# SiyuanHuang95/SUG

Measured on AMD Instinct MI355X. Metric: point-clouds/sec (train step, N=1024), higher is better.
Workload: dtype f32

## Files before the change

include/sug_amd.h:

```cpp
#ifndef SUG_AMD_H
#define SUG_AMD_H

#include <stdint.h>

#ifdef __cplusplus
extern "C" {
#endif

#define SUG_OK 0
#define SUG_ERR_ARG (-1)
#define SUG_ERR_LAUNCH (-2)
#define SUG_STATS_BLOCKS 1024

const char* sug_last_error(void);
#define SUG_ABI_VERSION 7
int sug_abi_version(void);

int sug_knn(const float* x, int64_t ldx, int B, int N, int C, int k,
            int32_t* idx, void* stream);

int sug_knn_reverse(const int32_t* idx, int B, int N, int k,
                    int32_t* rev_off, int32_t* rev_ent, void* stream);

int sug_fps(const float* xyz, const int32_t* start, int B, int N, int npoint,
            int32_t* out, void* stream);

int sug_ball_query(const float* xyz, const float* query, int B, int N, int S,
                   float r2, int nsample, int32_t* out, void* stream);

int sug_knn_query(const float* xyz, const float* query, int B, int N, int S,
                  int k, int32_t* idx_out, float* dist_out, void* stream);
int sug_knn_query_direct(const float* xyz, const float* query, int B, int N, int S, int k,
                         int32_t* idx_out, float* dist_out, void* stream);

int sug_three_nn(const float* query, const float* cand, int B, int N, int S,
                 int32_t* idx3, float* dist3, void* stream);

// ... 158 lines not shown
                           float eps, float momentum, float slope, float* running_mean,
                           float* running_var, float* z, uint8_t* arg, float* s1, float* coef,
                           float* out, int64_t ldo, double* stats, float* ws, void* stream);
int sug_edgeconv_fused_supported(int N, int k, int Cin, int Co);
int sug_edgeconv_fused_layer_fwd(const float* x, int64_t ldx, int Cin, const float* wcat, const float* qbias,
                                 const int32_t* idx, const float* gamma, const float* beta, int B, int N, int k,
                                 int Co, int groups, int training, float eps, float momentum, float slope,
                                 float* running_mean, float* running_var, float* z, uint8_t* arg, float* s1,
                                 float* pq_out, int64_t ldpq, float* coef, float* out, int64_t ldo, float* ws,
                                 void* stream);
int sug_edgeconv_layer_bwd(const float* gout, int64_t ldg, const float* z, const uint8_t* arg,
                           const float* s1, const float* pq, int64_t ldpq, const int32_t* idx,
                           const float* coef, int B, int N, int k, int Co, int groups, int training,
                           float slope, float* a, double* red, int32_t* rev_off, int32_t* rev_ent,
                           float* dpq, int64_t lddpq, float* ws, float* dgb, void* stream);
int sug_sa_first_fwd(const float* P, int64_t ldp, const float* Q, const int32_t* idx, int B, int N, int S,
                     int ns, int C, int groups, const float* gamma, const float* beta, int training,
                     float eps, float momentum, float* running_mean, float* running_var, float* coef,
                     float* Z, float* ws, void* stream);
int sug_sa_first_bwd(const float* gz, const float* P, int64_t ldp, const float* Q, const int32_t* idx, int B,
                     int N, int S, int ns, int C, int groups, int training, const float* coef, double* red,
                     int32_t* rev_off, int32_t* rev_ent, float* segsum, float* dP, float* dQ, float* ws, float* dgb,
                     void* stream);
int sug_sa_first_geo_fwd(const float* Pf, int64_t ldp, const float* xyz, const float* cent, const float* Wx, int ldw,
                         const float* bias, const int32_t* idx, int B, int N, int S, int ns, int C, int groups,
                         const float* gamma, const float* beta, int training, float eps, float momentum,
                         float* running_mean, float* running_var, float* coef, float* Z, float* ws, void* stream);
int sug_sa_first_geo_bwd(const float* gz, const float* Pf, int64_t ldp, const float* xyz, const float* cent, const float* Wx,
                         int ldw, const float* bias, const int32_t* idx, int B, int N, int S, int ns, int C, int groups,
                         int training, const float* coef, double* red, int32_t* rev_off, int32_t* rev_ent, float* segsum,
// ... 179 lines not shown
```

sug_amd/_lib.py:

```python
import ctypes
import os

import torch

_HERE = os.path.dirname(os.path.abspath(__file__))
LIB_PATH = os.path.join(_HERE, 'libsug_amd.so')

_vp, _i32, _i64, _f32, _f64 = ctypes.c_void_p, ctypes.c_int, ctypes.c_int64, ctypes.c_float, ctypes.c_double

SIGNATURES = {
    'sug_knn': [_vp, _i64, _i32, _i32, _i32, _i32, _vp, _vp],
    'sug_knn_reverse': [_vp, _i32, _i32, _i32, _vp, _vp, _vp],
    'sug_fps': [_vp, _vp, _i32, _i32, _i32, _vp, _vp],
    'sug_ball_query': [_vp, _vp, _i32, _i32, _i32, _f32, _i32, _vp, _vp],
    'sug_knn_query': [_vp, _vp, _i32, _i32, _i32, _i32, _vp, _vp, _vp],
    'sug_knn_query_direct': [_vp, _vp, _i32, _i32, _i32, _i32, _vp, _vp, _vp],
    'sug_three_nn': [_vp, _vp, _i32, _i32, _i32, _vp, _vp, _vp],
    'sug_three_nn_direct': [_vp, _vp, _i32, _i32, _i32, _vp, _vp, _vp],
    'sug_ball_query_multi': [_vp, _vp, _i32, _i32, _i32, _i32, _vp, _vp, _vp, _vp],
    'sug_fp_interp_fwd': [_vp, _i64, _vp, _vp, _i32, _i32, _i32, _i32, _vp, _i64, _vp, _vp],
    'sug_fp_interp_bwd': [_vp, _i64, _vp, _vp, _i32, _i32, _i32, _i32, _vp, _vp, _vp, _i64, _vp],
    'sug_gather_rows': [_vp, _i64, _vp, _i32, _i32, _i32, _i32, _vp, _i64, _vp],
    'sug_scatter_add_rows': [_vp, _i64, _vp, _i32, _i32, _i32, _i32, _vp, _i64, _vp],
    'sug_scatter_rows_ordered_supported': [_i32, _i32, _i32],
    'sug_scatter_rows_ordered': [_vp, _i64, _vp, _i32, _i32, _i32, _i32, _vp, _i64, _vp, _vp],
    'sug_group_max': [_vp, _i64, _vp, _i32, _i32, _i32, _i32, _i32, _vp, _vp, _vp],
    'sug_group_max_bwd': [_vp, _vp, _i32, _i32, _i32, _i32, _vp, _i64, _vp],
    'sug_edgeconv_fwd': [_vp, _i64, _vp, _vp, _i32, _i32, _i32, _i32, _vp, _vp, _vp, _vp, _vp, _vp],
    'sug_bn_finalize': [_vp, _vp, _vp, _i32, _f64, _f32, _f32, _vp, _vp, _vp, _vp],
    'sug_affine_act': [_vp, _i64, _vp, _i64, _i32, _f32, _vp, _i64, _vp],
    'sug_col_stats': [_vp, _i64, _i64, _i32, _vp, _vp, _vp],
    'sug_edgeconv_bwd_reduce': [_vp, _i64, _vp, _vp, _i64, _i32, _f32, _vp, _vp, _vp, _vp],
    'sug_edgeconv_bwd_scatter': [_vp, _vp, _vp, _vp, _i64, _vp, _vp, _vp, _vp, _i32, _i32, _i32, _i32,
                                 _vp, _i64, _vp],
    'sug_edgeconv_layer_fwd': [_vp, _i64, _vp, _vp, _vp, _i32, _i32, _i32, _i32, _i32, _i32, _f32, _f32, _f32, _vp, _vp,
                               _vp, _vp, _vp, _vp, _vp, _i64, _vp, _vp, _vp],
    'sug_edgeconv_fused_layer_fwd': [_vp, _i64, _i32, _vp, _vp, _vp, _vp, _vp, _i32, _i32, _i32, _i32, _i32, _i32, _f32, _f32, _f32,
                                     _vp, _vp, _vp, _vp, _vp, _vp, _i64, _vp, _vp, _i64, _vp, _vp],
    'sug_edgeconv_fused_supported': [_i32, _i32, _i32, _i32],
    'sug_edgeconv_layer_bwd': [_vp, _i64, _vp, _vp, _vp, _vp, _i64, _vp, _vp, _i32, _i32, _i32, _i32, _i32, _i32, _f32,
                               _vp, _vp, _vp, _vp, _vp, _i64, _vp, _vp, _vp],
    'sug_bn_act_rows_fwd': [_vp, _i64, _i64, _i32, _i32, _vp, _vp, _i32, _f32, _f32, _f32, _vp, _vp, _vp, _vp, _i64,
                            _vp, _vp, _vp],
    'sug_bn_act_rows_bwd': [_vp, _i64, _vp, _i64, _vp, _i64, _i32, _i32, _i32, _f32, _vp, _vp, _vp, _vp, _vp, _vp],
    'sug_bn_act_pool_layer_fwd': [_vp, _i64, _i32, _i32, _i32, _i32, _vp, _vp, _i32, _f32, _f32, _f32, _vp, _vp, _vp,
                                  _vp, _vp, _i64, _vp, _vp, _vp, _vp, _vp],
    'sug_bn_act_pool_layer_bwd': [_vp, _i64, _vp, _vp, _vp, _i64, _vp, _i32, _i32, _i32, _i32, _f32, _i32, _vp, _vp, _vp,
                                  _i64, _vp, _vp],
    'sug_fold_groups': [_vp, _i32, _i32, _vp, _vp],
    'sug_edgeconv_fwd_bn': [_vp, _i64, _vp, _vp, _vp, _i32, _i32, _i32, _i32, _f32, _f32, _vp, _vp, _vp, _vp, _vp, _vp,
                            _vp, _vp],
    'sug_col_stats_bn': [_vp, _i64, _i64, _i32, _vp, _vp, _f32, _f32, _vp, _vp, _vp, _vp, _vp],
    'sug_col_stats_bn_grouped': [_vp, _i64, _i64, _i32, _i32, _vp, _vp, _f32, _f32, _vp, _vp, _vp, _vp, _vp],
    'sug_bn_replay': [_vp, _i32, _i32, _f32, _vp, _vp, _vp],
    'sug_bn_replay_multi': [_i32, _vp, _vp, _vp, _vp, _vp, _vp, _vp],
    'sug_ptran_pos1_fwd': [_vp, _vp, _vp, _vp, _i32, _i32, _i32, _i32, _i32, _vp, _vp],
# ... 140 lines not shown
```

sug_amd/csrc/edgeconv.hip:

```cpp
#include "common.h"

namespace {

__device__ __forceinline__ float4 ld4(const float* p) { return *reinterpret_cast<const float4*>(p); }
__device__ __forceinline__ void st4(float* p, float4 v) { *reinterpret_cast<float4*>(p) = v; }

template <int NCH>
__global__ __launch_bounds__(256) void edgeconv_fwd_kernel(
    const float* __restrict__ pq, int64_t ldpq, const int32_t* __restrict__ idx,
    const float* __restrict__ gamma, int64_t BN, int N, int k, int Co, int LPP, int bpc,
    float* __restrict__ z, uint8_t* __restrict__ arg, float* __restrict__ s1,
    float* __restrict__ ws) {
  extern __shared__ __attribute__((aligned(16))) float s_red[];
  const int nchunk = Co >> 2;
  const int ppb = 256 / LPP;
  const int slot = threadIdx.x / LPP, ch0 = threadIdx.x % LPP;
  float4 a1[NCH], a2[NCH], gs[NCH];
#pragma unroll
  for (int u = 0; u < NCH; ++u) {
    a1[u] = make_float4(0, 0, 0, 0);
    a2[u] = make_float4(0, 0, 0, 0);
    const int ch = ch0 + u * LPP;
    gs[u] = ch < nchunk ? ld4(gamma + ch * 4) : make_float4(1, 1, 1, 1);
  }
// ... 651 lines not shown
      dP.x = ax - cf * (fx * dbx + hx * (pm.x - mean.x));
      dP.y = ay - cf * (fy * dby + hy * (pm.y - mean.y));
      dP.z = az - cf * (fz * dbz + hz * (pm.z - mean.z));
      dP.w = aw - cf * (fw * dbw + hw * (pm.w - mean.w));
      const float4 ap = ld4(a + p * Co + c), sp = ld4(s1 + p * Co + c);
      dQ.x = ap.x - (kf * fx * dbx + hx * (sp.x - kf * mean.x));
      dQ.y = ap.y - (kf * fy * dby + hy * (sp.y - kf * mean.y));
      dQ.z = ap.z - (kf * fz * dbz + hz * (sp.z - kf * mean.z));
      dQ.w = ap.w - (kf * fw * dbw + hw * (sp.w - kf * mean.w));
      st4(dpq + p * lddpq + c, dP);
      st4(dpq + p * lddpq + Co + c, dQ);
    }
  }
}

template <int SW, int KK>
__global__ __launch_bounds__(1024) void edgeconv_bwd_lds_kernel(
    const float* __restrict__ a, const uint8_t* __restrict__ arg, const float* __restrict__ s1,
    const float* __restrict__ pq, int64_t ldpq, const int32_t* __restrict__ rev_off,
    const int32_t* __restrict__ rev_ent, const float* __restrict__ coef_all, const double* __restrict__ red_all,
    int B, int N, int Co, int psplit, float invM, int Bg, int64_t coef_stride, int64_t red_stride,
    float* __restrict__ dpq, int64_t lddpq) {
  extern __shared__ __attribute__((aligned(16))) float s_lds[];
  constexpr int LP = SW / 4;
  constexpr int PPP = 1024 / LP;
  float* s_a = s_lds;
  float* s_q = s_lds + (size_t)N * SW;
  uint32_t* s_g = reinterpret_cast<uint32_t*>(s_q + (size_t)N * SW);
  int* s_hist = reinterpret_cast<int*>(s_g + (size_t)N * LP);
  uint16_t* s_perm = reinterpret_cast<uint16_t*>(s_hist + 512);
  const int nslice = Co / SW;
  const int per_cloud = nslice * psplit;
  int b, r;
  if ((B & 7) == 0) {
    const int xcd = blockIdx.x & 7, j = blockIdx.x >> 3;
    b = (j / per_cloud) * 8 + xcd;
    r = j % per_cloud;
  } else {
    b = blockIdx.x / per_cloud;
    r = blockIdx.x % per_cloud;
  }
  const int sl = r % nslice, part = r / nslice;
  const int c0 = sl * SW;
  const int64_t rowb = (int64_t)b * N;
  const float* coef = coef_all + (int64_t)(b / Bg) * coef_stride;
  const double* red = red_all + (int64_t)(b / Bg) * red_stride;
  for (int e = threadIdx.x; e < N * LP; e += 1024) {
    const int n = e / LP, c4 = e % LP;
    const int64_t o = (rowb + n) * Co + c0 + c4 * 4;
    st4(s_a + n * SW + c4 * 4, ld4(a + o));
    st4(s_q + n * SW + c4 * 4, ld4(pq + (rowb + n) * ldpq + Co + c0 + c4 * 4));
    s_g[n * LP + c4] = *reinterpret_cast<const uint32_t*>(arg + o);
  }
  const int32_t* offb = rev_off + (int64_t)b * (N + 1);
  if (threadIdx.x < 256) s_hist[threadIdx.x] = 0;
  __syncthreads();
  for (int m = part + psplit * (int)threadIdx.x; m < N; m += psplit * 1024) {
    const int c = offb[m + 1] - offb[m];
    atomicAdd(&s_hist[255 - (c < 255 ? c : 255)], 1);
  }
  __syncthreads();
  {
    int* scr = s_hist + 256;
    const int mine = threadIdx.x < 256 ? s_hist[threadIdx.x] : 0;
    if (threadIdx.x < 256) scr[threadIdx.x] = mine;
    __syncthreads();
    for (int o = 1; o < 256; o <<= 1) {
      int t = 0;
      if (threadIdx.x < 256 && threadIdx.x >= o) t = scr[threadIdx.x - o];
      __syncthreads();
      if (threadIdx.x < 256) scr[threadIdx.x] += t;
      __syncthreads();
    }
    if (threadIdx.x < 256) s_hist[threadIdx.x] = scr[threadIdx.x] - mine;
    __syncthreads();
  }
  for (int m = part + psplit * (int)threadIdx.x; m < N; m += psplit * 1024) {
    const int c = offb[m + 1] - offb[m];
    s_perm[atomicAdd(&s_hist[255 - (c < 255 ? c : 255)], 1)] = (uint16_t)m;
  }
  const int n_own = (N - part + psplit - 1) / psplit;
  const int lp = threadIdx.x % LP, slot = threadIdx.x / LP;
  const int c = c0 + lp * 4;
  const float4 sc = ld4(coef + c), mean = ld4(coef + 2 * Co + c), rstd = ld4(coef + 3 * Co + c);
  const float dbx = (float)red[c + 0], dby = (float)red[c + 1], dbz = (float)red[c + 2], dbw = (float)red[c + 3];
  const float dgx = (float)red[Co + c + 0], dgy = (float)red[Co + c + 1];
  const float dgz = (float)red[Co + c + 2], dgw = (float)red[Co + c + 3];
  const float fx = sc.x * invM, fy = sc.y * invM, fz = sc.z * invM, fw = sc.w * invM;
  const float hx = fx * rstd.x * dgx, hy = fy * rstd.y * dgy, hz = fz * rstd.z * dgz, hw = fw * rstd.w * dgw;
  const float kf = (float)KK;
  const int32_t* entb = rev_ent + (int64_t)b * N * KK;
  __syncthreads();
  for (int pos = slot; pos < n_own; pos += PPP) {
    const int m = s_perm[pos];
    const int off = offb[m], cnt = offb[m + 1] - off;
    const int32_t* ent = entb + off;
    float ax = 0, ay = 0, az = 0, aw = 0, qx = 0, qy = 0, qz = 0, qw = 0;
    constexpr int GB = 8;
    for (int t0 = 0; t0 < cnt; t0 += GB) {
      int en[GB];
#pragma unroll
      for (int t = 0; t < GB; ++t) en[t] = (t0 + t < cnt) ? ent[t0 + t] : -1;
#pragma unroll
      for (int t = 0; t < GB; ++t) {
        if (en[t] >= 0) {
          const int n = en[t] / KK, j = en[t] - n * KK;
          const float4 av = ld4(s_a + n * SW + lp * 4), qv = ld4(s_q + n * SW + lp * 4);
          const uint32_t g = s_g[n * LP + lp];
          ax += (int)(g & 255u) == j ? av.x : 0.f;
          ay += (int)((g >> 8) & 255u) == j ? av.y : 0.f;
          az += (int)((g >> 16) & 255u) == j ? av.z : 0.f;
          aw += (int)(g >> 24) == j ? av.w : 0.f;
          qx += qv.x; qy += qv.y; qz += qv.z; qw += qv.w;
        }
      }
    }
    const int64_t p = rowb + m;
    const float4 pm = ld4(pq + p * ldpq + c);
    const float cf = (float)cnt;
    float4 dP, dQ;
    dP.x = ax - (hx * qx + cf * (fx * dbx + hx * (pm.x - mean.x)));
// ... 300 lines not shown

extern "C" int sug_edgeconv_bwd_reduce(const float* gout, int64_t ldg, const float* z, const float* coef,
                                       int64_t rows, int Co, float slope, float* a, double* red,
                                       float* ws, void* stream) {
  SUG_REQUIRE(gout && z && coef && a && red && ws, "sug_edgeconv_bwd_reduce: null pointer");
  SUG_REQUIRE(rows > 0 && Co > 0 && Co <= 4096 && ldg >= Co, "sug_edgeconv_bwd_reduce: bad shape");
  hipStream_t st = (hipStream_t)stream;
  const int grid = launch_col_reduce<1>(gout, ldg, z, coef, rows, Co, slope, a, ws, st);
  SUG_LAUNCH_CHECK("sug_edgeconv_bwd_reduce");
  hipLaunchKernelGGL(reduce_partials_kernel, dim3(sug_divup(2 * Co, 16)), dim3(256), 0, st, ws, grid, 2 * Co, red);
  SUG_LAUNCH_CHECK("sug_edgeconv_bwd_reduce(reduce)");
  return SUG_OK;
}

static int edgeconv_bwd_scatter_groups(const float* a, const uint8_t* arg, const float* s1, const float* pq,
                                       int64_t ldpq, const int32_t* rev_off, const int32_t* rev_ent, const float* coef,
                                       const double* red, int B, int N, int k, int Co, int groups, int64_t coef_stride,
                                       int64_t red_stride, float* dpq, int64_t lddpq, void* stream);

extern "C" int sug_edgeconv_bwd_scatter(const float* a, const uint8_t* arg, const float* s1,
                                        const float* pq, int64_t ldpq, const int32_t* rev_off,
                                        const int32_t* rev_ent, const float* coef, const double* red,
                                        int B, int N, int k, int Co, float* dpq, int64_t lddpq,
                                        void* stream) {
  return edgeconv_bwd_scatter_groups(a, arg, s1, pq, ldpq, rev_off, rev_ent, coef, red, B, N, k, Co, 1, 0, 0, dpq, lddpq,
                                     stream);
}

int sug_edgeconv_bwd_scatter_groups(const float* a, const uint8_t* arg, const float* s1, const float* pq, int64_t ldpq,
                                    const int32_t* rev_off, const int32_t* rev_ent, const float* coef, const double* red,
                                    int B, int N, int k, int Co, int groups, int64_t coef_stride, int64_t red_stride,
                                    float* dpq, int64_t lddpq, void* stream) {
  return edgeconv_bwd_scatter_groups(a, arg, s1, pq, ldpq, rev_off, rev_ent, coef, red, B, N, k, Co, groups, coef_stride,
                                     red_stride, dpq, lddpq, stream);
}

static int edgeconv_bwd_scatter_groups(const float* a, const uint8_t* arg, const float* s1, const float* pq,
                                       int64_t ldpq, const int32_t* rev_off, const int32_t* rev_ent, const float* coef,
                                       const double* red, int B, int N, int k, int Co, int groups, int64_t coef_stride,
                                       int64_t red_stride, float* dpq, int64_t lddpq, void* stream) {
  SUG_REQUIRE(a && arg && s1 && pq && rev_off && rev_ent && coef && red && dpq,
              "sug_edgeconv_bwd_scatter: null pointer");
  SUG_REQUIRE(B > 0 && N > 0 && k > 0 && k <= 255, "sug_edgeconv_bwd_scatter: bad shape");
  SUG_REQUIRE(groups >= 1 && B % groups == 0, "sug_edgeconv_bwd_scatter: B=%d does not split into %d groups", B, groups);
  SUG_REQUIRE(Co > 0 && Co % 4 == 0 && Co <= 1024, "sug_edgeconv_bwd_scatter: Co=%d", Co);
  SUG_REQUIRE(ldpq >= 2 * Co && ldpq % 4 == 0 && lddpq >= 2 * Co && lddpq % 4 == 0,
              "sug_edgeconv_bwd_scatter: bad row strides");
  const int Bg = B / groups;
  const int64_t BN = (int64_t)Bg * N;
  const float invM = (float)(1.0 / ((double)BN * k));
  hipStream_t st = (hipStream_t)stream;
#ifndef SUG_EDGECONV_NO_LDS
  const size_t sh_lds = (size_t)N * 16 * 9 + 512 * sizeof(int) + (size_t)N * sizeof(uint16_t);
  if (k == 20 && Co % 16 == 0 && N <= 65535 && sh_lds <= 158 * 1024 && !getenv("SUG_EDGECONV_BWD_LEGACY") &&
      ((uintptr_t)a % 16) == 0 && ((uintptr_t)pq % 16) == 0 && ((uintptr_t)arg % 4) == 0 && ((uintptr_t)dpq % 16) == 0 &&
      ((uintptr_t)s1 % 16) == 0 && ((uintptr_t)coef % 16) == 0) {
    const int nslice = Co / 16;
    int psplit = 256 / (B * nslice);
    psplit = psplit < 1 ? 1 : (psplit > 4 ? 4 : psplit);
    static SugLdsOptIn note;
    if (int rc = sug_allow_dynamic_lds(note, &edgeconv_bwd_lds_kernel<16, 20>, 158 * 1024, "sug_edgeconv_bwd_scatter(lds)")) return rc;
    hipLaunchKernelGGL((edgeconv_bwd_lds_kernel<16, 20>), dim3(B * nslice * psplit), dim3(1024), sh_lds, st, a, arg, s1, pq,
                       ldpq, rev_off, rev_ent, coef, red, B, N, Co, psplit, invM, Bg, coef_stride, red_stride, dpq, lddpq);
    SUG_LAUNCH_CHECK("sug_edgeconv_bwd_scatter(lds)");
    return SUG_OK;
  }
#endif
  const int lpp = lanes_per_point(Co);
  const int nch = sug_divup(Co >> 2, lpp);
  const int ppb = 256 / lpp;
  const int cpx = sug_divup(Bg, 8);
  int bpc = sug_divup(N, ppb);
  while (bpc > 1 && (int64_t)8 * cpx * bpc > 8192) bpc = (bpc + 1) / 2;
  const int grid = 8 * cpx * bpc;
#define LAUNCH_SCATTER(NC) do { \
    if (k == 20) hipLaunchKernelGGL((edgeconv_bwd_scatter_kernel<NC, 20>), dim3(grid), dim3(256), 0, st, ag, argg, s1g, pqg, ldpq, offg, entg, cg, rg, BN, N, k, Co, lpp, bpc, invM, dpqg, lddpq); \
    else hipLaunchKernelGGL((edgeconv_bwd_scatter_kernel<NC, 0>), dim3(grid), dim3(256), 0, st, ag, argg, s1g, pqg, ldpq, offg, entg, cg, rg, BN, N, k, Co, lpp, bpc, invM, dpqg, lddpq); \
  } while (0)
// ... 40 lines not shown
```

sug_amd/csrc/knn.hip:

```cpp
#include "common.h"

namespace {

template <int K>
__device__ __forceinline__ void topk_insert_desc(float (&v)[K], int (&id)[K], float s, int j) {
#pragma unroll
  for (int t = K - 1; t > 0; --t) {
    const bool up = s > v[t - 1];
    const bool here = s > v[t];
    const float nv = up ? v[t - 1] : (here ? s : v[t]);
    const int ni = up ? id[t - 1] : (here ? j : id[t]);
    v[t] = nv;
    id[t] = ni;
  }
  if (s > v[0]) {
    v[0] = s;
    id[0] = j;
  }
}

template <int C>
struct TileStride { static constexpr int value = (C % 4 == 0) ? C + 4 : C; };

template <int C, int K, int BLOCK, int TJ>
// ... 151 lines not shown
      else if (TJ == 32)
        hipLaunchKernelGGL((knn_self_generic_kernel<K, BLOCK, 32>), grid, dim3(BLOCK), sh, st, x, ldx, N, C, k, idx);
      else if (TJ == 16)
        hipLaunchKernelGGL((knn_self_generic_kernel<K, BLOCK, 16>), grid, dim3(BLOCK), sh, st, x, ldx, N, C, k, idx);
      else
        hipLaunchKernelGGL((knn_self_generic_kernel<K, BLOCK, 8>), grid, dim3(BLOCK), (size_t)8 * C * sizeof(float), st, x, ldx, N, C, k, idx);
      SUG_LAUNCH_CHECK("sug_knn(generic)");
      return SUG_OK;
    }
  }
}

template <int BLOCK>
__global__ __launch_bounds__(BLOCK) void knn_reverse_kernel(const int32_t* __restrict__ idx, int N,
                                                            int E, int RS, int sorted, int32_t* __restrict__ rev_off,
                                                            int32_t* __restrict__ rev_ent) {
  extern __shared__ int s_i[];
  constexpr int NW = BLOCK / 64;
  const int Nr = (N + RS - 1) / RS;
  int* cnt = s_i;
  int* cur = s_i + Nr;
  int* scr = s_i + 2 * Nr;
  int* ent = s_i + 2 * Nr + 2 * NW;
  const int b = blockIdx.x / RS, r = blockIdx.x % RS;
  const int lo = r * Nr, hi = (lo + Nr < N) ? lo + Nr : N;
  const int nr = hi > lo ? hi - lo : 0;
  const int lane = threadIdx.x & 63, wave = threadIdx.x >> 6;
  const int32_t* ib = idx + (int64_t)b * E;
  int32_t* off = rev_off + (int64_t)b * (N + 1);
  int32_t* gent = rev_ent + (int64_t)b * E;
  for (int i = threadIdx.x; i < nr; i += BLOCK) cnt[i] = 0;
// ... 85 lines not shown
    if (n <= 32) continue;
    const int s = cur[i] - n;
    for (int u = lane; u < n; u += 64) {
      const int key = ent[s + u];
      int rank = 0;
      for (int j0 = 0; j0 < n; j0 += 8) {
        int v[8];
#pragma unroll
        for (int t = 0; t < 8; ++t) v[t] = ent[s + min(j0 + t, n - 1)];
#pragma unroll
        for (int t = 0; t < 8; ++t) rank += (j0 + t < n && v[t] < key) ? 1 : 0;
      }
      gent[base + s + rank] = key;
    }
  }
}

}

extern "C" int sug_knn(const float* x, int64_t ldx, int B, int N, int C, int k, int32_t* idx,
                       void* stream) {
  SUG_REQUIRE(x && idx, "sug_knn: null pointer");
  SUG_REQUIRE(B > 0 && N > 0 && C > 0, "sug_knn: bad shape B=%d N=%d C=%d", B, N, C);
  SUG_REQUIRE(k >= 1 && k <= 32 && k <= N, "sug_knn: need 1 <= k <= min(32,N), got k=%d N=%d", k, N);
  SUG_REQUIRE(ldx >= C, "sug_knn: ldx=%lld < C=%d", (long long)ldx, C);
  SUG_REQUIRE(B <= 65535, "sug_knn: B=%d exceeds grid.y", B);
  hipStream_t st = (hipStream_t)stream;
  if (sug_knn_pc_supported(x, ldx, C, k)) return sug_knn_pc(x, ldx, B, N, C, k, idx, st);
  if (k <= 16) return dispatch_knn_c<16>(x, ldx, B, N, C, k, idx, st);
  if (k <= 20) return dispatch_knn_c<20>(x, ldx, B, N, C, k, idx, st);
  return dispatch_knn_c<32>(x, ldx, B, N, C, k, idx, st);
}

size_t sug_reverse_lists_lds_bytes(int B, int E, int N, int* ranges) {
  int RS = 1;
  while (RS < 8 && B * RS < 256 && N / (RS * 2) >= 64) RS *= 2;
  const int Nr = (N + RS - 1) / RS;
  if (ranges) *ranges = RS;
  return (size_t)(2 * Nr + 2 * (1024 / 64) + (size_t)E) * sizeof(int);
}

int sug_reverse_lists(const int32_t* idx, int B, int E, int N, int sorted, int32_t* rev_off, int32_t* rev_ent,
                      hipStream_t st) {
  SUG_REQUIRE(idx && rev_off && rev_ent, "sug_reverse_lists: null pointer");
  SUG_REQUIRE(B > 0 && N > 0 && E > 0, "sug_reverse_lists: bad shape");
  constexpr int BLOCK = 1024;
  int RS = 0;
  const size_t sh = sug_reverse_lists_lds_bytes(B, E, N, &RS);
  SUG_REQUIRE(sh <= 160 * 1024, "sug_reverse_lists: %d entries per cloud are too many for the LDS-resident build", E);
  static SugLdsOptIn note;
  if (int rc = sug_allow_dynamic_lds(note, &knn_reverse_kernel<BLOCK>, 160 * 1024, "sug_reverse_lists")) return rc;
  hipLaunchKernelGGL((knn_reverse_kernel<BLOCK>), dim3(B * RS), dim3(BLOCK), sh, st, idx, N, E, RS, sorted, rev_off,
                     rev_ent);
  SUG_LAUNCH_CHECK("sug_reverse_lists");
  return SUG_OK;
}

extern "C" int sug_knn_reverse(const int32_t* idx, int B, int N, int k, int32_t* rev_off,
                               int32_t* rev_ent, void* stream) {
  SUG_REQUIRE(B > 0 && N > 0 && k > 0, "sug_knn_reverse: bad shape");
  return sug_reverse_lists(idx, B, N * k, N, 1, rev_off, rev_ent, (hipStream_t)stream);
}
```

sug_amd/csrc/layers.cpp:

```cpp
#include <stdint.h>
#include "../../include/sug_amd.h"

void sug_set_error(const char* fmt, ...);
struct ihipStream_t;
int sug_col_stats_bn_groups(const float* y, int64_t ldy, int64_t rows, int C, int groups, const float* gamma,
                            const float* beta, float eps, float momentum, float* running_mean, float* running_var,
                            float* coef, float* ws, ihipStream_t* st);
int sug_affine_act_groups(const float* z, int64_t ldz, const float* coef, int64_t rows, int groups, int C, float slope,
                          float* out, int64_t ldo, ihipStream_t* st);
int sug_bwd_reduce_groups(const float* gout, int64_t ldg, const float* z, const float* coef, int64_t rows, int Co,
                          int groups, float slope, float* a, double* red, float* ws, ihipStream_t* st, float* dgb);
int sug_bn_bwd_apply_groups(const float* a, int64_t lda, int from_g, float slope, const float* y, int64_t ldy,
                            const float* coef, const double* red, int64_t rows_g, int groups, int C, float* dy,
                            int64_t lddy, ihipStream_t* st);
int sug_edgeconv_fwd_bn_act_groups(const float* pq, int64_t ldpq, const int32_t* idx, const float* gamma,
                                   const float* beta, int B, int N, int k, int Co, int groups, float eps, float momentum,
                                   float slope, float* running_mean, float* running_var, float* z, uint8_t* arg,
                                   float* s1, float* coef, float* out, int64_t ldo, float* ws, void* stream);
int sug_edgeconv_bwd_scatter_groups(const float* a, const uint8_t* arg, const float* s1, const float* pq, int64_t ldpq,
                                    const int32_t* rev_off, const int32_t* rev_ent, const float* coef, const double* red,
                                    int B, int N, int k, int Co, int groups, int64_t coef_stride, int64_t red_stride,
                                    float* dpq, int64_t lddpq, void* stream);
#define LAYER_REQUIRE(cond, ...) do { if (!(cond)) { sug_set_error(__VA_ARGS__); return SUG_ERR_ARG; } } while (0)
#define LAYER_TRY(call) do { const int rc_ = (call); if (rc_ != SUG_OK) return rc_; } while (0)

extern "C" int sug_edgeconv_layer_fwd(const float* pq, int64_t ldpq, const int32_t* idx, const float* gamma,
                                      const float* beta, int B, int N, int k, int Co, int groups, int training,
                                      float eps, float momentum, float slope, float* running_mean,
                                      float* running_var, float* z, uint8_t* arg, float* s1, float* coef,
                                      float* out, int64_t ldo, double* stats, float* ws, void* stream) {
  LAYER_REQUIRE(groups >= 1 && B > 0 && B % groups == 0, "sug_edgeconv_layer_fwd: B=%d does not split into %d groups", B, groups);
  LAYER_REQUIRE(coef && out && z && arg && stats, "sug_edgeconv_layer_fwd: null pointer");
  const int Bg = B / groups;
  const int64_t rows = (int64_t)Bg * N;
  if (training)
    return sug_edgeconv_fwd_bn_act_groups(pq, ldpq, idx, gamma, beta, B, N, k, Co, groups, eps, momentum, slope, running_mean,
                                          running_var, z, arg, s1, coef, out, ldo, ws, stream);
  for (int g = 0; g < groups; ++g) {
    const int64_t r0 = (int64_t)g * rows;
    float* cg = coef + (int64_t)g * 5 * Co;
    LAYER_TRY(sug_edgeconv_fwd(pq + r0 * ldpq, ldpq, idx + r0 * k, gamma, Bg, N, k, Co, z + r0 * Co, arg + r0 * Co,
                               s1 ? s1 + r0 * Co : nullptr, stats, ws, stream));
    LAYER_TRY(sug_affine_act(z + r0 * Co, Co, cg, rows, Co, slope, out + r0 * ldo, ldo, stream));
  }
  return SUG_OK;
}

extern "C" int sug_edgeconv_layer_bwd(const float* gout, int64_t ldg, const float* z, const uint8_t* arg,
                                      const float* s1, const float* pq, int64_t ldpq, const int32_t* idx,
                                      const float* coef, int B, int N, int k, int Co, int groups, int training,
                                      float slope, float* a, double* red, int32_t* rev_off, int32_t* rev_ent,
                                      float* dpq, int64_t lddpq, float* ws, float* dgb, void* stream) {
  LAYER_REQUIRE(groups >= 1 && B > 0 && B % groups == 0, "sug_edgeconv_layer_bwd: B=%d does not split into %d groups", B, groups);
  LAYER_REQUIRE(red && a && rev_off && rev_ent, "sug_edgeconv_layer_bwd: null pointer");
  const int Bg = B / groups;
  const int64_t rows = (int64_t)Bg * N;
  LAYER_TRY(sug_knn_reverse(idx, B, N, k, rev_off, rev_ent, stream));
  int grouped = 1;
  if (groups > 1) {
    grouped = sug_bwd_reduce_groups(gout, ldg, z, coef, rows, Co, groups, slope, a, red, ws, (ihipStream_t*)stream, dgb);
    if (grouped < 0) return grouped;
  }
  for (int g = 0; grouped != 0 && g < groups; ++g) {
    const int64_t r0 = (int64_t)g * rows;
    const float* cg = coef + (int64_t)g * 5 * Co;
    double* rg = red + (int64_t)g * 2 * Co;
    LAYER_TRY(sug_edgeconv_bwd_reduce(gout + r0 * ldg, ldg, z + r0 * Co, cg, rows, Co, slope, a + r0 * Co, rg, ws, stream));
  }
  LAYER_TRY(sug_edgeconv_bwd_scatter_groups(a, arg, s1, pq, ldpq, rev_off, rev_ent, coef,
                                            training ? red : red + (int64_t)groups * 2 * Co, B, N, k, Co, groups,
                                            (int64_t)5 * Co, training ? (int64_t)2 * Co : 0, dpq, lddpq, stream));
  if (dgb && grouped != 0) LAYER_TRY(sug_fold_groups(red, groups, 2 * Co, dgb, stream));
  return SUG_OK;
}

extern "C" int sug_bn_act_rows_fwd(const float* y, int64_t ldy, int64_t rows, int C, int groups,
                                   const float* gamma, const float* beta, int training, float eps, float momentum,
                                   float slope, float* running_mean, float* running_var, float* coef, float* out,
                                   int64_t ldo, double* stats, float* ws, void* stream) {
  LAYER_REQUIRE(groups >= 1 && rows > 0 && rows % groups == 0, "sug_bn_act_rows_fwd: %lld rows do not split into %d groups",
                (long long)rows, groups);
  LAYER_REQUIRE(coef && out, "sug_bn_act_rows_fwd: null pointer");
  const int64_t rg = rows / groups;
  ihipStream_t* st = (ihipStream_t*)stream;
// ... 119 lines not shown
```

sug_amd/ops.py:

```python
import contextlib
import ctypes
import math
import os as _os

import torch

from ._lib import lib, check, STATS_BLOCKS

class StepContext:
    __slots__ = ('bn_groups', 'start_queue', 'start_provider', 'geometry_plan', 'profile', 'profile_only', 'parallel_branches',
                 'fused_heads', 'w16_cache', 'bn_record', 'pending_counts')

    def __init__(self):
        self.bn_groups = 1
        self.start_queue = self.start_provider = self.geometry_plan = None
        self.profile = self.profile_only = None
        self.parallel_branches = False
        self.fused_heads = False
        self.w16_cache = self.bn_record = self.pending_counts = None


CTX = StepContext()

SIGMA_LIST = (0.01, 0.1, 1, 10, 100)
# ... 1149 lines not shown
    C = y.shape[-1]
    pooled = bn_act_pool_cat(y, bn, slope)
    return pooled[:, :C], pooled[:, C:]


def _edgeconv_out(out_holder, B, N, Co, dev):
    if out_holder is None:
        return torch.empty(B, N, Co, dtype=torch.float32, device=dev)
    out = out_holder[0]
    if tuple(out.shape) != (B, N, Co) or out.stride(2) != 1 or out.stride(0) != N * out.stride(1) \
            or out.dtype != torch.float32 or out.requires_grad:
        raise RuntimeError('edgeconv: bad destination slice')
    return out


def _edgeconv_backward(gout, z, arg, s1, pq, ldpq, idx, coef, B, N, k, Co, G, slope, train):
    dev = gout.device
    gout, _, _, _, ldg = _rows3(gout)
    a = torch.empty(B, N, Co, dtype=torch.float32, device=dev)
    red = (torch.empty if train else torch.zeros)(G + 1, 2 * Co, dtype=torch.float64, device=dev)
    ws = _stats_ws(Co, dev)
    off = torch.empty(B, N + 1, dtype=torch.int32, device=dev)
    ent = torch.empty(B, N * k, dtype=torch.int32, device=dev)
    dpq = torch.empty(B, N, 2 * Co, dtype=torch.float32, device=dev)
    rf = torch.empty(2 * Co, dtype=torch.float32, device=dev)
    check(_timed('edgeconv_layer_bwd_Co%d' % Co, {'B': B, 'N': N, 'k': k, 'Co': Co},
                 lambda: lib().sug_edgeconv_layer_bwd(_p(gout), ldg, _p(z), _p(arg), _p(s1), _p(pq), ldpq, _p(idx),
                                                      _p(coef), B, N, k, Co, G, train, slope, _p(a),
                                                      _p(red), _p(off), _p(ent), _p(dpq), 2 * Co, _p(ws), _p(rf), _st())),
          'sug_edgeconv_layer_bwd')
    return (dpq,) + _dgamma_dbeta(rf)


class _EdgeConv(torch.autograd.Function):

    @staticmethod
    def forward(ctx, pq, idx, gamma, beta, st, slope, out_holder, grad_on=True):
        _need_gpu(pq, idx, gamma)
        pq, B, N, C2, ld = _rows3(pq)
        Co = C2 // 2
        idx = _i32(idx).contiguous()
        k = idx.shape[2]
        G = st.G
        _check_groups('edgeconv', B, 'clouds', G)
        dev = pq.device
# ... 1464 lines not shown
```

Before: 13580.

## Precompute reverse-list visiting order in knn_reverse and use DPP-shared entry loads in edgeconv bwd

Moves the per-block histogram/prefix-scan sort of points by reverse-list length out of the edgeconv backward LDS kernel and into the reverse-list builder, which now emits a 16-bit descending-count order. The scatter kernel reads this order, alternates slot direction on each pass to even out per-wave load, and loads reverse entries as aligned int2 pairs shared across a quad via DPP broadcasts. Entries are pre-packed as (n<<8)|j, so the per-entry integer division goes away. The trade-offs are extra rank-counting work in the reverse kernel, a new order buffer, and an added 8-byte alignment requirement on rev_ent.

Result: no change. 13490 (-0.6%).

```diff
diff --git a/include/sug_amd.h b/include/sug_amd.h
--- a/include/sug_amd.h
+++ b/include/sug_amd.h
@@ -21,6 +21,8 @@
 
 int sug_knn_reverse(const int32_t* idx, int B, int N, int k,
                     int32_t* rev_off, int32_t* rev_ent, void* stream);
+int sug_knn_reverse_ord(const int32_t* idx, int B, int N, int k,
+                        int32_t* rev_off, int32_t* rev_ent, uint16_t* rev_ord, void* stream);
 
 int sug_fps(const float* xyz, const int32_t* start, int B, int N, int npoint,
             int32_t* out, void* stream);
@@ -209,6 +211,11 @@
                            const float* coef, int B, int N, int k, int Co, int groups, int training,
                            float slope, float* a, double* red, int32_t* rev_off, int32_t* rev_ent,
                            float* dpq, int64_t lddpq, float* ws, float* dgb, void* stream);
+int sug_edgeconv_layer_bwd_ord(const float* gout, int64_t ldg, const float* z, const uint8_t* arg,
+                               const float* s1, const float* pq, int64_t ldpq, const int32_t* idx,
+                               const float* coef, int B, int N, int k, int Co, int groups, int training,
+                               float slope, float* a, double* red, int32_t* rev_off, int32_t* rev_ent,
+                               uint16_t* rev_ord, float* dpq, int64_t lddpq, float* ws, float* dgb, void* stream);
 int sug_sa_first_fwd(const float* P, int64_t ldp, const float* Q, const int32_t* idx, int B, int N, int S,
                      int ns, int C, int groups, const float* gamma, const float* beta, int training,
                      float eps, float momentum, float* running_mean, float* running_var, float* coef,
diff --git a/sug_amd/_lib.py b/sug_amd/_lib.py
--- a/sug_amd/_lib.py
+++ b/sug_amd/_lib.py
@@ -11,6 +11,7 @@
 SIGNATURES = {
     'sug_knn': [_vp, _i64, _i32, _i32, _i32, _i32, _vp, _vp],
     'sug_knn_reverse': [_vp, _i32, _i32, _i32, _vp, _vp, _vp],
+    'sug_knn_reverse_ord': [_vp, _i32, _i32, _i32, _vp, _vp, _vp, _vp],
     'sug_fps': [_vp, _vp, _i32, _i32, _i32, _vp, _vp],
     'sug_ball_query': [_vp, _vp, _i32, _i32, _i32, _f32, _i32, _vp, _vp],
     'sug_knn_query': [_vp, _vp, _i32, _i32, _i32, _i32, _vp, _vp, _vp],
@@ -40,6 +41,8 @@
     'sug_edgeconv_fused_supported': [_i32, _i32, _i32, _i32],
     'sug_edgeconv_layer_bwd': [_vp, _i64, _vp, _vp, _vp, _vp, _i64, _vp, _vp, _i32, _i32, _i32, _i32, _i32, _i32, _f32,
                                _vp, _vp, _vp, _vp, _vp, _i64, _vp, _vp, _vp],
+    'sug_edgeconv_layer_bwd_ord': [_vp, _i64, _vp, _vp, _vp, _vp, _i64, _vp, _vp, _i32, _i32, _i32, _i32, _i32, _i32, _f32,
+                                   _vp, _vp, _vp, _vp, _vp, _vp, _i64, _vp, _vp, _vp],
     'sug_bn_act_rows_fwd': [_vp, _i64, _i64, _i32, _i32, _vp, _vp, _i32, _f32, _f32, _f32, _vp, _vp, _vp, _vp, _i64,
                             _vp, _vp, _vp],
     'sug_bn_act_rows_bwd': [_vp, _i64, _vp, _i64, _vp, _i64, _i32, _i32, _i32, _f32, _vp, _vp, _vp, _vp, _vp, _vp],
diff --git a/sug_amd/csrc/edgeconv.hip b/sug_amd/csrc/edgeconv.hip
--- a/sug_amd/csrc/edgeconv.hip
+++ b/sug_amd/csrc/edgeconv.hip
@@ -689,21 +689,26 @@
   }
 }
 
+template <int Q>
+__device__ __forceinline__ int quad_bcast(int v) {
+  return __builtin_amdgcn_update_dpp(0, v, Q * 0x55, 0xF, 0xF, false);
+}
+
 template <int SW, int KK>
 __global__ __launch_bounds__(1024) void edgeconv_bwd_lds_kernel(
     const float* __restrict__ a, const uint8_t* __restrict__ arg, const float* __restrict__ s1,
     const float* __restrict__ pq, int64_t ldpq, const int32_t* __restrict__ rev_off,
-    const int32_t* __restrict__ rev_ent, const float* __restrict__ coef_all, const double* __restrict__ red_all,
-    int B, int N, int Co, int psplit, float invM, int Bg, int64_t coef_stride, int64_t red_stride,
-    float* __restrict__ dpq, int64_t lddpq) {
+    const int32_t* __restrict__ rev_ent, const uint16_t* __restrict__ ord, const float* __restrict__ coef_all,
+    const double* __restrict__ red_all, int B, int N, int Co, int psplit, float invM, int Bg, int64_t coef_stride,
+    int64_t red_stride, float* __restrict__ dpq, int64_t lddpq) {
   extern __shared__ __attribute__((aligned(16))) float s_lds[];
+  static_assert(SW == 16 && KK % 2 == 0, "4 lanes per point fetch 8 entries; a cloud's entries start 8-byte aligned");
   constexpr int LP = SW / 4;
   constexpr int PPP = 1024 / LP;
+  constexpr int PPW = 64 / LP;
   float* s_a = s_lds;
   float* s_q = s_lds + (size_t)N * SW;
   uint32_t* s_g = reinterpret_cast<uint32_t*>(s_q + (size_t)N * SW);
-  int* s_hist = reinterpret_cast<int*>(s_g + (size_t)N * LP);
-  uint16_t* s_perm = reinterpret_cast<uint16_t*>(s_hist + 512);
   const int nslice = Co / SW;
   const int per_cloud = nslice * psplit;
   int b, r;
@@ -728,34 +733,10 @@
     s_g[n * LP + c4] = *reinterpret_cast<const uint32_t*>(arg + o);
   }
   const int32_t* offb = rev_off + (int64_t)b * (N + 1);
-  if (threadIdx.x < 256) s_hist[threadIdx.x] = 0;
-  __syncthreads();
-  for (int m = part + psplit * (int)threadIdx.x; m < N; m += psplit * 1024) {
-    const int c = offb[m + 1] - offb[m];
-    atomicAdd(&s_hist[255 - (c < 255 ? c : 255)], 1);
-  }
-  __syncthreads();
-  {
-    int* scr = s_hist + 256;
-    const int mine = threadIdx.x < 256 ? s_hist[threadIdx.x] : 0;
-    if (threadIdx.x < 256) scr[threadIdx.x] = mine;
-    __syncthreads();
-    for (int o = 1; o < 256; o <<= 1) {
-      int t = 0;
-      if (threadIdx.x < 256 && threadIdx.x >= o) t = scr[threadIdx.x - o];
-      __syncthreads();
-      if (threadIdx.x < 256) scr[threadIdx.x] += t;
-      __syncthreads();
-    }
-    if (threadIdx.x < 256) s_hist[threadIdx.x] = scr[threadIdx.x] - mine;
-    __syncthreads();
-  }
-  for (int m = part + psplit * (int)threadIdx.x; m < N; m += psplit * 1024) {
-    const int c = offb[m + 1] - offb[m];
-    s_perm[atomicAdd(&s_hist[255 - (c < 255 ? c : 255)], 1)] = (uint16_t)m;
-  }
+  const uint16_t* ordb = ord ? ord + rowb : nullptr;
   const int n_own = (N - part + psplit - 1) / psplit;
   const int lp = threadIdx.x % LP, slot = threadIdx.x / LP;
+  const int slot_rev = (PPP - PPW - (slot / PPW) * PPW) + slot % PPW;
   const int c = c0 + lp * 4;
   const float4 sc = ld4(coef + c), mean = ld4(coef + 2 * Co + c), rstd = ld4(coef + 3 * Co + c);
   const float dbx = (float)red[c + 0], dby = (float)red[c + 1], dbz = (float)red[c + 2], dbw = (float)red[c + 3];
@@ -766,20 +747,34 @@
   const float kf = (float)KK;
   const int32_t* entb = rev_ent + (int64_t)b * N * KK;
   __syncthreads();
-  for (int pos = slot; pos < n_own; pos += PPP) {
-    const int m = s_perm[pos];
+  for (int p0 = 0, pass = 0; p0 < n_own; p0 += PPP, ++pass) {
+    const int pos = p0 + ((pass & 1) ? slot_rev : slot);
+    if (pos >= n_own) continue;
+    const int at = part + psplit * pos;
+    const int m = ordb ? (int)ordb[at] : at;
     const int off = offb[m], cnt = offb[m + 1] - off;
-    const int32_t* ent = entb + off;
+    const int lead = off & 1, tot = cnt + lead;
+    const int32_t* ent = entb + (off - lead);
     float ax = 0, ay = 0, az = 0, aw = 0, qx = 0, qy = 0, qz = 0, qw = 0;
     constexpr int GB = 8;
-    for (int t0 = 0; t0 < cnt; t0 += GB) {
+    for (int t0 = 0; t0 < tot; t0 += GB) {
+      const int s = t0 + 2 * lp;
+      int2 e2 = make_int2(-1, -1);
+      if (s < tot) e2 = *reinterpret_cast<const int2*>(ent + s);
+      if (s < lead) e2.x = -1;
+      if (s + 1 >= tot) e2.y = -1;
+      const int n0 = e2.x / KK, n1 = e2.y / KK;
+      const int d0 = e2.x < 0 ? -1 : (n0 << 8) | (e2.x - n0 * KK);
+      const int d1 = e2.y < 0 ? -1 : (n1 << 8) | (e2.y - n1 * KK);
       int en[GB];
-#pragma unroll
-      for (int t = 0; t < GB; ++t) en[t] = (t0 + t < cnt) ? ent[t0 + t] : -1;
+      en[0] = quad_bcast<0>(d0); en[1] = quad_bcast<0>(d1);
+      en[2] = quad_bcast<1>(d0); en[3] = quad_bcast<1>(d1);
+      en[4] = quad_bcast<2>(d0); en[5] = quad_bcast<2>(d1);
+      en[6] = quad_bcast<3>(d0); en[7] = quad_bcast<3>(d1);
 #pragma unroll
       for (int t = 0; t < GB; ++t) {
         if (en[t] >= 0) {
-          const int n = en[t] / KK, j = en[t] - n * KK;
+          const int n = en[t] >> 8, j = en[t] & 255;
           const float4 av = ld4(s_a + n * SW + lp * 4), qv = ld4(s_q + n * SW + lp * 4);
           const uint32_t g = s_g[n * LP + lp];
           ax += (int)(g & 255u) == j ? av.x : 0.f;
@@ -1110,31 +1105,33 @@
 }
 
 static int edgeconv_bwd_scatter_groups(const float* a, const uint8_t* arg, const float* s1, const float* pq,
-                                       int64_t ldpq, const int32_t* rev_off, const int32_t* rev_ent, const float* coef,
-                                       const double* red, int B, int N, int k, int Co, int groups, int64_t coef_stride,
-                                       int64_t red_stride, float* dpq, int64_t lddpq, void* stream);
+                                       int64_t ldpq, const int32_t* rev_off, const int32_t* rev_ent,
+                                       const uint16_t* rev_ord, const float* coef, const double* red, int B, int N, int k,
+                                       int Co, int groups, int64_t coef_stride, int64_t red_stride, float* dpq,
+                                       int64_t lddpq, void* stream);
 
 extern "C" int sug_edgeconv_bwd_scatter(const float* a, const uint8_t* arg, const float* s1,
                                         const float* pq, int64_t ldpq, const int32_t* rev_off,
                                         const int32_t* rev_ent, const float* coef, const double* red,
                                         int B, int N, int k, int Co, float* dpq, int64_t lddpq,
                                         void* stream) {
-  return edgeconv_bwd_scatter_groups(a, arg, s1, pq, ldpq, rev_off, rev_ent, coef, red, B, N, k, Co, 1, 0, 0, dpq, lddpq,
-                                     stream);
+  return edgeconv_bwd_scatter_groups(a, arg, s1, pq, ldpq, rev_off, rev_ent, nullptr, coef, red, B, N, k, Co, 1, 0, 0, dpq,
+                                     lddpq, stream);
 }
 
 int sug_edgeconv_bwd_scatter_groups(const float* a, const uint8_t* arg, const float* s1, const float* pq, int64_t ldpq,
-                                    const int32_t* rev_off, const int32_t* rev_ent, const float* coef, const double* red,
-                                    int B, int N, int k, int Co, int groups, int64_t coef_stride, int64_t red_stride,
-                                    float* dpq, int64_t lddpq, void* stream) {
-  return edgeconv_bwd_scatter_groups(a, arg, s1, pq, ldpq, rev_off, rev_ent, coef, red, B, N, k, Co, groups, coef_stride,
-                                     red_stride, dpq, lddpq, stream);
+                                    const int32_t* rev_off, const int32_t* rev_ent, const uint16_t* rev_ord,
+                                    const float* coef, const double* red, int B, int N, int k, int Co, int groups,
+                                    int64_t coef_stride, int64_t red_stride, float* dpq, int64_t lddpq, void* stream) {
+  return edgeconv_bwd_scatter_groups(a, arg, s1, pq, ldpq, rev_off, rev_ent, rev_ord, coef, red, B, N, k, Co, groups,
+                                     coef_stride, red_stride, dpq, lddpq, stream);
 }
 
 static int edgeconv_bwd_scatter_groups(const float* a, const uint8_t* arg, const float* s1, const float* pq,
-                                       int64_t ldpq, const int32_t* rev_off, const int32_t* rev_ent, const float* coef,
-                                       const double* red, int B, int N, int k, int Co, int groups, int64_t coef_stride,
-                                       int64_t red_stride, float* dpq, int64_t lddpq, void* stream) {
+                                       int64_t ldpq, const int32_t* rev_off, const int32_t* rev_ent,
+                                       const uint16_t* rev_ord, const float* coef, const double* red, int B, int N, int k,
+                                       int Co, int groups, int64_t coef_stride, int64_t red_stride, float* dpq,
+                                       int64_t lddpq, void* stream) {
   SUG_REQUIRE(a && arg && s1 && pq && rev_off && rev_ent && coef && red && dpq,
               "sug_edgeconv_bwd_scatter: null pointer");
   SUG_REQUIRE(B > 0 && N > 0 && k > 0 && k <= 255, "sug_edgeconv_bwd_scatter: bad shape");
@@ -1147,17 +1144,17 @@
   const float invM = (float)(1.0 / ((double)BN * k));
   hipStream_t st = (hipStream_t)stream;
 #ifndef SUG_EDGECONV_NO_LDS
-  const size_t sh_lds = (size_t)N * 16 * 9 + 512 * sizeof(int) + (size_t)N * sizeof(uint16_t);
+  const size_t sh_lds = (size_t)N * 16 * 9;
   if (k == 20 && Co % 16 == 0 && N <= 65535 && sh_lds <= 158 * 1024 && !getenv("SUG_EDGECONV_BWD_LEGACY") &&
       ((uintptr_t)a % 16) == 0 && ((uintptr_t)pq % 16) == 0 && ((uintptr_t)arg % 4) == 0 && ((uintptr_t)dpq % 16) == 0 &&
-      ((uintptr_t)s1 % 16) == 0 && ((uintptr_t)coef % 16) == 0) {
+      ((uintptr_t)s1 % 16) == 0 && ((uintptr_t)coef % 16) == 0 && ((uintptr_t)rev_ent % 8) == 0) {
     const int nslice = Co / 16;
     int psplit = 256 / (B * nslice);
     psplit = psplit < 1 ? 1 : (psplit > 4 ? 4 : psplit);
     static SugLdsOptIn note;
     if (int rc = sug_allow_dynamic_lds(note, &edgeconv_bwd_lds_kernel<16, 20>, 158 * 1024, "sug_edgeconv_bwd_scatter(lds)")) return rc;
     hipLaunchKernelGGL((edgeconv_bwd_lds_kernel<16, 20>), dim3(B * nslice * psplit), dim3(1024), sh_lds, st, a, arg, s1, pq,
-                       ldpq, rev_off, rev_ent, coef, red, B, N, Co, psplit, invM, Bg, coef_stride, red_stride, dpq, lddpq);
+                       ldpq, rev_off, rev_ent, rev_ord, coef, red, B, N, Co, psplit, invM, Bg, coef_stride, red_stride, dpq, lddpq);
     SUG_LAUNCH_CHECK("sug_edgeconv_bwd_scatter(lds)");
     return SUG_OK;
   }
diff --git a/sug_amd/csrc/knn.hip b/sug_amd/csrc/knn.hip
--- a/sug_amd/csrc/knn.hip
+++ b/sug_amd/csrc/knn.hip
@@ -189,7 +189,7 @@
 template <int BLOCK>
 __global__ __launch_bounds__(BLOCK) void knn_reverse_kernel(const int32_t* __restrict__ idx, int N,
                                                             int E, int RS, int sorted, int32_t* __restrict__ rev_off,
-                                                            int32_t* __restrict__ rev_ent) {
+                                                            int32_t* __restrict__ rev_ent, uint16_t* __restrict__ ord) {
   extern __shared__ int s_i[];
   constexpr int NW = BLOCK / 64;
   const int Nr = (N + RS - 1) / RS;
@@ -305,6 +305,24 @@
       gent[base + s + rank] = key;
     }
   }
+  if (ord == nullptr) return;
+  __syncthreads();
+  uint32_t* key = reinterpret_cast<uint32_t*>(cur);
+  for (int i = threadIdx.x; i < nr; i += BLOCK) key[i] = ((uint32_t)cnt[i] << 16) | (uint32_t)(65535 - i);
+  __syncthreads();
+  int S = 1;
+  while (S < 64 && S * 2 * nr <= BLOCK) S *= 2;
+  const int sub = threadIdx.x & (S - 1), ipb = BLOCK / S;
+  uint16_t* ob = ord + (int64_t)b * N + lo;
+  for (int i0 = 0; i0 < nr; i0 += ipb) {
+    const int i = i0 + (int)threadIdx.x / S;
+    const uint32_t mine = i < nr ? key[i] : 0u;
+    int rank = 0;
+#pragma unroll 8
+    for (int j = sub; j < nr; j += S) rank += key[j] > mine ? 1 : 0;
+    for (int o = 1; o < S; o <<= 1) rank += __shfl_xor(rank, o);
+    if (i < nr && sub == 0) ob[rank] = (uint16_t)(lo + i);
+  }
 }
 
 }
@@ -331,10 +349,11 @@
   return (size_t)(2 * Nr + 2 * (1024 / 64) + (size_t)E) * sizeof(int);
 }
 
-int sug_reverse_lists(const int32_t* idx, int B, int E, int N, int sorted, int32_t* rev_off, int32_t* rev_ent,
-                      hipStream_t st) {
+static int reverse_lists(const int32_t* idx, int B, int E, int N, int sorted, int32_t* rev_off, int32_t* rev_ent,
+                         uint16_t* ord, hipStream_t st) {
   SUG_REQUIRE(idx && rev_off && rev_ent, "sug_reverse_lists: null pointer");
   SUG_REQUIRE(B > 0 && N > 0 && E > 0, "sug_reverse_lists: bad shape");
+  SUG_REQUIRE(!ord || (N <= 65535 && E <= 65535), "sug_reverse_lists: N=%d, E=%d too large for a 16-bit visiting order", N, E);
   constexpr int BLOCK = 1024;
   int RS = 0;
   const size_t sh = sug_reverse_lists_lds_bytes(B, E, N, &RS);
@@ -342,9 +361,14 @@
   static SugLdsOptIn note;
   if (int rc = sug_allow_dynamic_lds(note, &knn_reverse_kernel<BLOCK>, 160 * 1024, "sug_reverse_lists")) return rc;
   hipLaunchKernelGGL((knn_reverse_kernel<BLOCK>), dim3(B * RS), dim3(BLOCK), sh, st, idx, N, E, RS, sorted, rev_off,
-                     rev_ent);
+                     rev_ent, ord);
   SUG_LAUNCH_CHECK("sug_reverse_lists");
   return SUG_OK;
+}
+
+int sug_reverse_lists(const int32_t* idx, int B, int E, int N, int sorted, int32_t* rev_off, int32_t* rev_ent,
+                      hipStream_t st) {
+  return reverse_lists(idx, B, E, N, sorted, rev_off, rev_ent, nullptr, st);
 }
 
 extern "C" int sug_knn_reverse(const int32_t* idx, int B, int N, int k, int32_t* rev_off,
@@ -352,3 +376,9 @@
   SUG_REQUIRE(B > 0 && N > 0 && k > 0, "sug_knn_reverse: bad shape");
   return sug_reverse_lists(idx, B, N * k, N, 1, rev_off, rev_ent, (hipStream_t)stream);
 }
+
+extern "C" int sug_knn_reverse_ord(const int32_t* idx, int B, int N, int k, int32_t* rev_off,
+                                   int32_t* rev_ent, uint16_t* rev_ord, void* stream) {
+  SUG_REQUIRE(B > 0 && N > 0 && k > 0, "sug_knn_reverse_ord: bad shape");
+  return reverse_lists(idx, B, N * k, N, 1, rev_off, rev_ent, rev_ord, (hipStream_t)stream);
+}
diff --git a/sug_amd/csrc/layers.cpp b/sug_amd/csrc/layers.cpp
--- a/sug_amd/csrc/layers.cpp
+++ b/sug_amd/csrc/layers.cpp
@@ -18,9 +18,9 @@
                                    float slope, float* running_mean, float* running_var, float* z, uint8_t* arg,
                                    float* s1, float* coef, float* out, int64_t ldo, float* ws, void* stream);
 int sug_edgeconv_bwd_scatter_groups(const float* a, const uint8_t* arg, const float* s1, const float* pq, int64_t ldpq,
-                                    const int32_t* rev_off, const int32_t* rev_ent, const float* coef, const double* red,
-                                    int B, int N, int k, int Co, int groups, int64_t coef_stride, int64_t red_stride,
-                                    float* dpq, int64_t lddpq, void* stream);
+                                    const int32_t* rev_off, const int32_t* rev_ent, const uint16_t* rev_ord,
+                                    const float* coef, const double* red, int B, int N, int k, int Co, int groups,
+                                    int64_t coef_stride, int64_t red_stride, float* dpq, int64_t lddpq, void* stream);
 #define LAYER_REQUIRE(cond, ...) do { if (!(cond)) { sug_set_error(__VA_ARGS__); return SUG_ERR_ARG; } } while (0)
 #define LAYER_TRY(call) do { const int rc_ = (call); if (rc_ != SUG_OK) return rc_; } while (0)
 
@@ -51,11 +51,26 @@
                                       const float* coef, int B, int N, int k, int Co, int groups, int training,
                                       float slope, float* a, double* red, int32_t* rev_off, int32_t* rev_ent,
                                       float* dpq, int64_t lddpq, float* ws, float* dgb, void* stream) {
+  return sug_edgeconv_layer_bwd_ord(gout, ldg, z, arg, s1, pq, ldpq, idx, coef, B, N, k, Co, groups, training, slope, a, red,
+                                    rev_off, rev_ent, nullptr, dpq, lddpq, ws, dgb, stream);
+}
+
+extern "C" int sug_edgeconv_layer_bwd_ord(const float* gout, int64_t ldg, const float* z, const uint8_t* arg,
+                                          const float* s1, const float* pq, int64_t ldpq, const int32_t* idx,
+                                          const float* coef, int B, int N, int k, int Co, int groups, int training,
+                                          float slope, float* a, double* red, int32_t* rev_off, int32_t* rev_ent,
+                                          uint16_t* rev_ord, float* dpq, int64_t lddpq, float* ws, float* dgb,
+                                          void* stream) {
   LAYER_REQUIRE(groups >= 1 && B > 0 && B % groups == 0, "sug_edgeconv_layer_bwd: B=%d does not split into %d groups", B, groups);
   LAYER_REQUIRE(red && a && rev_off && rev_ent, "sug_edgeconv_layer_bwd: null pointer");
   const int Bg = B / groups;
   const int64_t rows = (int64_t)Bg * N;
-  LAYER_TRY(sug_knn_reverse(idx, B, N, k, rev_off, rev_ent, stream));
+  if (rev_ord && N <= 65535 && (int64_t)N * k <= 65535)
+    LAYER_TRY(sug_knn_reverse_ord(idx, B, N, k, rev_off, rev_ent, rev_ord, stream));
+  else {
+    LAYER_TRY(sug_knn_reverse(idx, B, N, k, rev_off, rev_ent, stream));
+    rev_ord = nullptr;
+  }
   int grouped = 1;
   if (groups > 1) {
     grouped = sug_bwd_reduce_groups(gout, ldg, z, coef, rows, Co, groups, slope, a, red, ws, (ihipStream_t*)stream, dgb);
@@ -67,7 +82,7 @@
     double* rg = red + (int64_t)g * 2 * Co;
     LAYER_TRY(sug_edgeconv_bwd_reduce(gout + r0 * ldg, ldg, z + r0 * Co, cg, rows, Co, slope, a + r0 * Co, rg, ws, stream));
   }
-  LAYER_TRY(sug_edgeconv_bwd_scatter_groups(a, arg, s1, pq, ldpq, rev_off, rev_ent, coef,
+  LAYER_TRY(sug_edgeconv_bwd_scatter_groups(a, arg, s1, pq, ldpq, rev_off, rev_ent, rev_ord, coef,
                                             training ? red : red + (int64_t)groups * 2 * Co, B, N, k, Co, groups,
                                             (int64_t)5 * Co, training ? (int64_t)2 * Co : 0, dpq, lddpq, stream));
   if (dgb && grouped != 0) LAYER_TRY(sug_fold_groups(red, groups, 2 * Co, dgb, stream));
diff --git a/sug_amd/ops.py b/sug_amd/ops.py
--- a/sug_amd/ops.py
+++ b/sug_amd/ops.py
@@ -1187,6 +1187,9 @@
     return out
 
 
+BWD_TAP = None
+
+
 def _edgeconv_backward(gout, z, arg, s1, pq, ldpq, idx, coef, B, N, k, Co, G, slope, train):
     dev = gout.device
     gout, _, _, _, ldg = _rows3(gout)
@@ -1195,13 +1198,17 @@
     ws = _stats_ws(Co, dev)
     off = torch.empty(B, N + 1, dtype=torch.int32, device=dev)
     ent = torch.empty(B, N * k, dtype=torch.int32, device=dev)
+    order = torch.empty(B, N, dtype=torch.int16, device=dev) if N * k <= 65535 else None
     dpq = torch.empty(B, N, 2 * Co, dtype=torch.float32, device=dev)
     rf = torch.empty(2 * Co, dtype=torch.float32, device=dev)
     check(_timed('edgeconv_layer_bwd_Co%d' % Co, {'B': B, 'N': N, 'k': k, 'Co': Co},
-                 lambda: lib().sug_edgeconv_layer_bwd(_p(gout), ldg, _p(z), _p(arg), _p(s1), _p(pq), ldpq, _p(idx),
-                                                      _p(coef), B, N, k, Co, G, train, slope, _p(a),
-                                                      _p(red), _p(off), _p(ent), _p(dpq), 2 * Co, _p(ws), _p(rf), _st())),
-          'sug_edgeconv_layer_bwd')
+                 lambda: lib().sug_edgeconv_layer_bwd_ord(_p(gout), ldg, _p(z), _p(arg), _p(s1), _p(pq), ldpq, _p(idx),
+                                                          _p(coef), B, N, k, Co, G, train, slope, _p(a),
+                                                          _p(red), _p(off), _p(ent), None if order is None else _p(order),
+                                                          _p(dpq), 2 * Co, _p(ws), _p(rf), _st())),
+          'sug_edgeconv_layer_bwd_ord')
+    if BWD_TAP is not None:
+        BWD_TAP.append((off, ent, order))
     return (dpq,) + _dgamma_dbeta(rf)
 
 
```
